# yangt1013/SPEINet

Hardware: AMD Instinct MI355X
Metric: deblurred 720p frames/sec (higher is better)
Workload: dtype f16 (correlation top2)

## Files before the change

speinet_amd/csrc/mlp_fused16.hip:

```cpp
#include "common.h"
#include <type_traits>

namespace {

constexpr int D = 256, HID = 512, MT = 128;
constexpr int RT = MT / 32;
constexpr int PA = 2 * D + 16;

template <typename LP>
struct MlpParams {
    const float* x;
    float* out;
    const LP* w1;
    const float* b1;
    const LP* w2;
    const float* b2;
    long long* stamps;
    int M;
};

typedef float f32x2 __attribute__((ext_vector_type(2)));

__device__ __forceinline__ f32x2 gelu2(f32x2 v) {
    const f32x2 u = v * v;
    f32x2 q = u * -1.419582270e-09f + 1.126438985e-07f;
    q = q * u + -3.898368825e-06f;
    q = q * u + 7.838465745e-05f;
    q = q * u + -1.034571474e-03f;
    q = q * u + 9.623637850e-03f;
    q = q * u + -6.612132016e-02f;
    q = q * u + 3.988274675e-01f;
    const f32x2 g = v * (v * q + 0.5f);
    f32x2 r;
    r[0] = fabsf(v[0]) < 4.0f ? g[0] : fmaxf(v[0], 0.f);
    r[1] = fabsf(v[1]) < 4.0f ? g[1] : fmaxf(v[1], 0.f);
    return r;
}

__device__ __forceinline__ f32x2 gelu2c(f32x2 v) {
    f32x2 c;
    c[0] = __builtin_amdgcn_fmed3f(v[0], -4.0f, 4.0f);
    c[1] = __builtin_amdgcn_fmed3f(v[1], -4.0f, 4.0f);
    const f32x2 u = c * c;
    f32x2 q = u * -1.419582270e-09f + 1.126438985e-07f;
    q = q * u + -3.898368825e-06f;
    q = q * u + 7.838465745e-05f;
    q = q * u + -1.034571474e-03f;
    q = q * u + 9.623637850e-03f;
    q = q * u + -6.612132016e-02f;
    q = q * u + 3.988274675e-01f;
    return v * (c * q + 0.5f);
}

struct GeluK { f32x2 c[8]; f32x2 half; };
__device__ __forceinline__ f32x2 sgpr_pair(float v) {
    f32x2 r = {v, v};
    asm volatile("" : "+s"(r));
    return r;
}
__device__ __forceinline__ GeluK gelu_consts() {
    GeluK k;
    k.c[0] = sgpr_pair(-1.419582270e-09f); k.c[1] = sgpr_pair(1.126438985e-07f); k.c[2] = sgpr_pair(-3.898368825e-06f);
    k.c[3] = sgpr_pair(7.838465745e-05f);  k.c[4] = sgpr_pair(-1.034571474e-03f); k.c[5] = sgpr_pair(9.623637850e-03f);
    k.c[6] = sgpr_pair(-6.612132016e-02f); k.c[7] = sgpr_pair(3.988274675e-01f);
    k.half = sgpr_pair(0.5f);
    return k;
}
__device__ __forceinline__ f32x4 gelu4c(f32x4 v, const GeluK& k) {
    const f32x2 va = {v[0], v[1]}, vb = {v[2], v[3]};
    f32x2 ca, cb;
    ca[0] = __builtin_amdgcn_fmed3f(v[0], -4.0f, 4.0f); ca[1] = __builtin_amdgcn_fmed3f(v[1], -4.0f, 4.0f);
    cb[0] = __builtin_amdgcn_fmed3f(v[2], -4.0f, 4.0f); cb[1] = __builtin_amdgcn_fmed3f(v[3], -4.0f, 4.0f);
    const f32x2 ua = ca * ca, ub = cb * cb;
    f32x2 qa = __builtin_elementwise_fma(ua, k.c[0], k.c[1]), qb = __builtin_elementwise_fma(ub, k.c[0], k.c[1]);
#pragma unroll
    for (int j = 2; j < 8; ++j) {
        qa = __builtin_elementwise_fma(qa, ua, k.c[j]);
        qb = __builtin_elementwise_fma(qb, ub, k.c[j]);
    }
    qa = __builtin_elementwise_fma(ca, qa, k.half);
    qb = __builtin_elementwise_fma(cb, qb, k.half);
    const f32x2 ga = va * qa, gb = vb * qb;
    return f32x4{ga[0], ga[1], gb[0], gb[1]};
}

template <int CTRL>
__device__ __forceinline__ float dpp_add(float v) { return v + dpp_quad<CTRL>(v); }
__device__ __forceinline__ float sum16(float v) { return dpp_add<0x140>(dpp_add<0x141>(dpp_add<0x4E>(dpp_add<0xB1>(v)))); }

template <typename LP>
__global__ __launch_bounds__(512) void mlp_fused_kernel(const MlpParams<LP> p) {
    typedef typename lpv<LP>::x8 lp8;
    typedef typename lpv<LP>::x4 lp4;
    constexpr int RG = 8;
    extern __shared__ __attribute__((aligned(16))) unsigned char smem[];
    unsigned char* sa = smem;
    unsigned char* sh = smem + MT * PA;
    float* bias1 = reinterpret_cast<float*>(smem + 2 * MT * PA);

    const int tid = threadIdx.x, lane = tid & 63, wave = tid >> 6;
    const int fr = lane & 31, fk = lane >> 5;
    const int m0 = blockIdx.x * MT;
    const int et = fr & 3, ecol = (fr >> 2) * 4;

    SPEI_STAMP(p.stamps, 0);
    bias1[tid] = p.b1[tid];
    const int rot = blockIdx.x & 15, rotb = rot * 32;

    {
        const int l16 = tid & 15, rsub = tid >> 4;
        f32x4 xr[MT / 32][4];
#pragma unroll
        for (int b = 0; b < MT / 32; ++b) {
            const int m = min(m0 + b * 32 + rsub, p.M - 1);
#pragma unroll
            for (int j = 0; j < 4; ++j) xr[b][j] = reinterpret_cast<const f32x4*>(p.x + (size_t)m * D)[l16 + 16 * j];
        }
#pragma unroll
        for (int b = 0; b < MT / 32; ++b) {
            const int r = b * 32 + rsub;
            float s = 0.f;
#pragma unroll
            for (int j = 0; j < 4; ++j) s += (xr[b][j][0] + xr[b][j][1]) + (xr[b][j][2] + xr[b][j][3]);
            const float mean = sum16(s) * (1.0f / 256.0f);
            float ss = 0.f;
#pragma unroll
            for (int j = 0; j < 4; ++j) {
                xr[b][j] -= mean;
                ss += (xr[b][j][0] * xr[b][j][0] + xr[b][j][1] * xr[b][j][1]) + (xr[b][j][2] * xr[b][j][2] + xr[b][j][3] * xr[b][j][3]);
            }
            const float rstd = 1.0f / sqrtf(sum16(ss) * (1.0f / 256.0f) + 1e-5f);
#pragma unroll
            for (int j = 0; j < 4; ++j) {
                lp4 hv;
#pragma unroll
                for (int e = 0; e < 4; ++e) hv[e] = to_lp<LP>(xr[b][j][e] * rstd);
                *reinterpret_cast<lp4*>(sa + r * PA + (((l16 + 16 * j) * 8 - rotb) & 511)) = hv;
            }
        }
    }

    lp8 ring[RG];
    const LP* wptr = p.w1 + (size_t)wave * 16 * 512 + lane * 8;
#pragma unroll
    for (int d = 0; d < RG; ++d) ring[d] = *reinterpret_cast<const lp8*>(wptr + ((rot + d) & 15) * 512);
    f32x4 res[RT][4];
#pragma unroll
    for (int i = 0; i < RT; ++i)
#pragma unroll
        for (int k = 0; k < 4; ++k) {
            const int m = min(m0 + i * 32 + 8 * k + 4 * fk + et, p.M - 1);
            res[i][k] = *reinterpret_cast<const f32x4*>(p.x + (size_t)m * D + wave * 32 + ecol);
        }
    __builtin_amdgcn_sched_barrier(0);
    lds_barrier();
    SPEI_STAMP(p.stamps, 1);

    f32x16 acc2[RT];
    const unsigned char* abase = sa + fr * PA + fk * 16;
    const unsigned char* hbase = sh + fr * PA + fk * 16;
#pragma unroll
    for (int half = 0; half < 2; ++half) {
        f32x16 acc1[RT];
#pragma unroll
        for (int g = 0; g < 4; ++g) {
            const f32x4 bv = *reinterpret_cast<const f32x4*>(bias1 + half * 256 + wave * 32 + 8 * g + 4 * fk);
#pragma unroll
            for (int i = 0; i < RT; ++i)
#pragma unroll
                for (int e = 0; e < 4; ++e) acc1[i][4 * g + e] = bv[e];
        }
        lp8 tn[RT];
#pragma unroll
        for (int i = 0; i < RT; ++i) tn[i] = *reinterpret_cast<const lp8*>(abase + i * 32 * PA);
        const LP* wnext = p.w2 + (size_t)wave * 32 * 512 + (size_t)half * 16 * 512 + lane * 8;
#pragma unroll
        for (int s = 0; s < 16; ++s) {
            lp8 tc[RT];
#pragma unroll
            for (int i = 0; i < RT; ++i) tc[i] = tn[i];
            if (s + 1 < 16) {
#pragma unroll
                for (int i = 0; i < RT; ++i) tn[i] = *reinterpret_cast<const lp8*>(abase + i * 32 * PA + (s + 1) * 32);
            }
            const lp8 w = ring[s % RG];
            ring[s % RG] = s + RG < 16 ? *reinterpret_cast<const lp8*>(wptr + ((rot + s + RG) & 15) * 512)
                                       : *reinterpret_cast<const lp8*>(wnext + ((rot + s + RG - 16) & 15) * 512);
            __builtin_amdgcn_sched_barrier(0);
#pragma unroll
            for (int i = 0; i < RT; ++i) acc1[i] = mfma16(w, tc[i], acc1[i]);
            __builtin_amdgcn_sched_barrier(0);
        }
        SPEI_STAMP(p.stamps, 2 + 3 * half);
        if (half == 0) {
            const float bias = p.b2[wave * 32 + fr];
#pragma unroll
            for (int i = 0; i < RT; ++i)
#pragma unroll
                for (int k = 0; k < 4; ++k) {
                    float a[4] = {res[i][k][0], res[i][k][1], res[i][k][2], res[i][k][3]};
                    quad_transpose4(a[0], a[1], a[2], a[3], et);
#pragma unroll
                    for (int e = 0; e < 4; ++e) acc2[i][4 * k + e] = a[e] + bias;
                }
        } else {
            lds_barrier();
        }
#pragma unroll
        for (int g = 0; g < 4; ++g) {
#pragma unroll
            for (int i = 0; i < RT; ++i) {
                const f32x2 g01 = gelu2c(f32x2{acc1[i][4 * g], acc1[i][4 * g + 1]});
                const f32x2 g23 = gelu2c(f32x2{acc1[i][4 * g + 2], acc1[i][4 * g + 3]});
                lp4 hv;
                hv[0] = to_lp<LP>(g01[0]); hv[1] = to_lp<LP>(g01[1]); hv[2] = to_lp<LP>(g23[0]); hv[3] = to_lp<LP>(g23[1]);
                *reinterpret_cast<lp4*>(sh + (i * 32 + fr) * PA + (((wave * 32 + 8 * g + 4 * fk) * 2 - rotb) & 511)) = hv;
            }
        }
        lds_barrier();
        SPEI_STAMP(p.stamps, 3 + 3 * half);
        wptr = wnext;
        const LP* wafter = p.w1 + (size_t)(8 + wave) * 16 * 512 + lane * 8;
#pragma unroll
        for (int i = 0; i < RT; ++i) tn[i] = *reinterpret_cast<const lp8*>(hbase + i * 32 * PA);
#pragma unroll
        for (int s = 0; s < 16; ++s) {
            lp8 tc[RT];
#pragma unroll
            for (int i = 0; i < RT; ++i) tc[i] = tn[i];
            if (s + 1 < 16) {
#pragma unroll
                for (int i = 0; i < RT; ++i) tn[i] = *reinterpret_cast<const lp8*>(hbase + i * 32 * PA + (s + 1) * 32);
            }
            const lp8 w = ring[s % RG];
            if (s + RG < 16) ring[s % RG] = *reinterpret_cast<const lp8*>(wptr + ((rot + s + RG) & 15) * 512);
            else if (half == 0) ring[s % RG] = *reinterpret_cast<const lp8*>(wafter + ((rot + s + RG - 16) & 15) * 512);
            __builtin_amdgcn_sched_barrier(0);
#pragma unroll
            for (int i = 0; i < RT; ++i) acc2[i] = mfma16(tc[i], w, acc2[i]);
            __builtin_amdgcn_sched_barrier(0);
        }
        SPEI_STAMP(p.stamps, 4 + 3 * half);
        wptr = wafter;
    }

#pragma unroll
    for (int i = 0; i < RT; ++i) {
#pragma unroll
        for (int k = 0; k < 4; ++k) {
            float a[4];
#pragma unroll
            for (int e = 0; e < 4; ++e) a[e] = acc2[i][4 * k + e];
            quad_transpose4(a[0], a[1], a[2], a[3], et);
            const int m = m0 + i * 32 + 8 * k + 4 * fk + et;
            if (m < p.M) *reinterpret_cast<f32x4*>(p.out + (size_t)m * D + wave * 32 + ecol) = f32x4{a[0], a[1], a[2], a[3]};
        }
    }
    SPEI_STAMP(p.stamps, 8);
}


constexpr int MP = 96;
constexpr int RP3 = MP / 32;
constexpr int SLABP = MP * PA;

template <typename LP>
__global__ __launch_bounds__(512) void mlp_pipe_kernel(const MlpParams<LP> p, const int ntiles, const int stagger) {
    typedef typename lpv<LP>::x8 lp8;
    typedef typename lpv<LP>::x4 lp4;
    constexpr int RG = 8;
    extern __shared__ __attribute__((aligned(16))) unsigned char smem[];
    unsigned char* const sb = smem + SLABP;
    float* bias1 = reinterpret_cast<float*>(smem + 3 * SLABP);

    const int tid = threadIdx.x, lane = tid & 63, wave = __builtin_amdgcn_readfirstlane(tid >> 6);
    const int fr = lane & 31, fk = lane >> 5;
    const int l16 = tid & 15, rsub = tid >> 4;

    SPEI_STAMP(p.stamps, 0); SPEI_STAMP_CLK(p.stamps, 8 + 0);
    spei_stagger_start(ntiles, stagger);
    bias1[tid] = p.b1[tid];
    const float bias2 = p.b2[wave * 32 + fr];
    const __amdgpu_buffer_rsrc_t rs1 = __builtin_amdgcn_make_buffer_rsrc(const_cast<LP*>(p.w1), 0, HID * D * 2, 0x00020000);
    const __amdgpu_buffer_rsrc_t rs2 = __builtin_amdgcn_make_buffer_rsrc(const_cast<LP*>(p.w2), 0, HID * D * 2, 0x00020000);
    const int lane16 = lane * 16;
    const int fbase[4] = {wave * 16, (8 + wave) * 16, wave * 32, wave * 32 + 16};
    auto wload = [&](int ph, int kstep) -> lp8 {
        return __builtin_bit_cast(lp8, __builtin_amdgcn_raw_buffer_load_b128(ph < 2 ? rs1 : rs2, lane16, (fbase[ph] + kstep) * 1024, 0));
    };

    const GeluK gk = gelu_consts();
    int tile = blockIdx.x;
    f32x4 xr[RP3][4];
    float lnm[RP3], lns[RP3];
    auto x_load = [&](int t, int b, int j) {
        const int m = min(t * MP + b * 32 + rsub, p.M - 1);
        xr[b][j] = reinterpret_cast<const f32x4*>(p.x + (size_t)m * D)[l16 + 16 * j];
    };
    auto ln_slice = [&](int b, int sub, unsigned char* dst, int rb) {
#pragma clang fp contract(off)
        if (sub == 0) {
            float s = 0.f;
#pragma unroll
            for (int j = 0; j < 4; ++j) s += (xr[b][j][0] + xr[b][j][1]) + (xr[b][j][2] + xr[b][j][3]);
            lnm[b] = sum16(s) * (1.0f / 256.0f);
        } else if (sub == 1) {
            float ss = 0.f;
#pragma unroll
            for (int j = 0; j < 4; ++j) {
                xr[b][j] -= lnm[b];
                ss += __builtin_fmaf(xr[b][j][1], xr[b][j][1], xr[b][j][0] * xr[b][j][0]) + __builtin_fmaf(xr[b][j][3], xr[b][j][3], xr[b][j][2] * xr[b][j][2]);
            }
            lns[b] = ss;
        } else if (sub == 2) {
            lns[b] = 1.0f / sqrtf(__builtin_fmaf(sum16(lns[b]), 1.0f / 256.0f, 1e-5f));
        } else {
            const int r = b * 32 + rsub;
#pragma unroll
            for (int j = 0; j < 4; ++j) {
                lp4 hv;
#pragma unroll
                for (int e = 0; e < 4; ++e) hv[e] = to_lp<LP>(xr[b][j][e] * lns[b]);
                *reinterpret_cast<lp4*>(dst + r * PA + (((l16 + 16 * j) * 8 - rb) & 511)) = hv;
            }
        }
    };

    int rot = tile & 15;
#pragma unroll
    for (int b = 0; b < RP3; ++b)
#pragma unroll
        for (int j = 0; j < 4; ++j) x_load(tile, b, j);
    lp8 ring[RG];
#pragma unroll
    for (int d = 0; d < RG; ++d) ring[d] = wload(0, (rot + d) & 15);
#pragma unroll
    for (int b = 0; b < RP3; ++b)
#pragma unroll
        for (int sub = 0; sub < 4; ++sub) ln_slice(b, sub, smem, rot * 32);
    __builtin_amdgcn_sched_barrier(0);
    lds_barrier();
    SPEI_STAMP(p.stamps, 1); SPEI_STAMP_CLK(p.stamps, 8 + 1);

    const unsigned range = (unsigned)p.M * (D * 4u);
    const __amdgpu_buffer_rsrc_t rsx = __builtin_amdgcn_make_buffer_rsrc(const_cast<float*>(p.x), 0, (int)range, 0x00020000);
    const __amdgpu_buffer_rsrc_t rso = __builtin_amdgcn_make_buffer_rsrc(p.out, 0, (int)range, 0x00020000);
    const unsigned voff_row = fk * 4096 + fr * 4;
    f32x16 acc2[RP3];
#pragma unroll
    for (int i = 0; i < RP3; ++i)
#pragma unroll
        for (int r = 0; r < 16; ++r) acc2[i][r] = 0.f;
    int cur = 0;
    bool first = true;
    for (; tile < ntiles; tile += gridDim.x) {
        unsigned char* const sa = smem + (cur ? 2 * SLABP : 0);
        unsigned char* const sc = smem + (cur ? 0 : 2 * SLABP);
        const int tnext = tile + gridDim.x;
        const int rotn = tnext & 15, rotb = rot * 32;
        auto wfrag = [&](int q) -> lp8 {
            return wload((q >> 4) & 3, ((q >= 64 ? rotn : rot) + (q & 15)) & 15);
        };
        auto gemm = [&](auto phc, const unsigned char* src, f32x16 (&acc)[RP3], auto weights_are_a, auto&& filler) {
            constexpr int ph = decltype(phc)::value;
            const unsigned char* base = src + fr * PA + fk * 16;
            lp8 tn[RP3];
#pragma unroll
            for (int i = 0; i < RP3; ++i) tn[i] = *reinterpret_cast<const lp8*>(base + i * 32 * PA);
#pragma unroll
            for (int s = 0; s < 16; ++s) {
                lp8 tc[RP3];
#pragma unroll
                for (int i = 0; i < RP3; ++i) tc[i] = tn[i];
                if (s + 1 < 16) {
#pragma unroll
                    for (int i = 0; i < RP3; ++i) tn[i] = *reinterpret_cast<const lp8*>(base + i * 32 * PA + (s + 1) * 32);
                }
                const lp8 w = ring[(ph * 16 + s) % RG];
                ring[(ph * 16 + s) % RG] = wfrag(ph * 16 + s + RG);
                __builtin_amdgcn_sched_barrier(0);
#pragma unroll
                for (int i = 0; i < RP3; ++i) {
                    if constexpr (decltype(weights_are_a)::value) acc[i] = mfma16(w, tc[i], acc[i]);
                    else acc[i] = mfma16(tc[i], w, acc[i]);
                }
                filler(s);
#pragma unroll
                for (int i = 0; i < RP3; ++i) asm volatile("" : "+v"(acc[i]));
                __builtin_amdgcn_sched_barrier(0);
            }
        };
        auto gelu_slice = [&](const f32x16 (&acc)[RP3], int s, unsigned char* dst) {
            if (s < 4 * RP3) {
                const int i = s >> 2, g = s & 3;
                const f32x4 gv = gelu4c(f32x4{acc[i][4 * g], acc[i][4 * g + 1], acc[i][4 * g + 2], acc[i][4 * g + 3]}, gk);
                *reinterpret_cast<lp4*>(dst + (i * 32 + fr) * PA + (((wave * 32 + 8 * g + 4 * fk) * 2 - rotb) & 511)) = to_lp4<LP>(gv);
            }
        };
        auto init_rows = [&](f32x16 (&acc)[RP3], const float* b) {
#pragma unroll
            for (int g = 0; g < 4; ++g) {
                const f32x4 bv = *reinterpret_cast<const f32x4*>(b + wave * 32 + 8 * g + 4 * fk);
#pragma unroll
                for (int i = 0; i < RP3; ++i)
#pragma unroll
                    for (int e = 0; e < 4; ++e) acc[i][4 * g + e] = bv[e];
            }
        };

        const unsigned vthis = voff_row + (unsigned)tile * (MP * 1024u), vprev = vthis - gridDim.x * (MP * 1024u);
        f32x16 acc1a[RP3], acc1b[RP3];
        f32x16 res[RP3];
        init_rows(acc1a, bias1);
        gemm(std::integral_constant<int, 0>{}, sa, acc1a, std::true_type{}, [&](int s) {
            if (s < 4 * RP3) {
                const int i = s >> 2, k = s & 3;
                const unsigned vst = vprev + (i * 32 + 8 * k) * 1024u, vld = vthis + (i * 32 + 8 * k) * 1024u;
#pragma unroll
                for (int e = 0; e < 4; ++e) {
                    __builtin_amdgcn_raw_buffer_store_b32(__float_as_uint(acc2[i][4 * k + e]), rso, (int)(vst + e * 1024u), wave * 128, 0);
                    res[i][4 * k + e] = __uint_as_float(__builtin_amdgcn_raw_buffer_load_b32(rsx, (int)(vld + e * 1024u), wave * 128, 0));
                }
            }
        });
        if (first) { SPEI_STAMP(p.stamps, 2); SPEI_STAMP_CLK(p.stamps, 8 + 2); }
        init_rows(acc1b, bias1 + 256);
        gemm(std::integral_constant<int, 1>{}, sa, acc1b, std::true_type{}, [&](int s) {
            gelu_slice(acc1a, s, sb);
            if (s >= 4 * RP3) {
#pragma unroll
                for (int i = 0; i < RP3; ++i)
#pragma unroll
                    for (int e = 0; e < 4; ++e) acc2[i][4 * (s - 4 * RP3) + e] = res[i][4 * (s - 4 * RP3) + e] + bias2;
            }
        });
        lds_barrier();
        if (first) { SPEI_STAMP(p.stamps, 3); SPEI_STAMP_CLK(p.stamps, 8 + 3); }
        gemm(std::integral_constant<int, 2>{}, sb, acc2, std::false_type{}, [&](int s) {
            gelu_slice(acc1b, s, sa);
            if (s >= 4 && (s & 3) < 2) {
                x_load(tnext, (s >> 2) - 1, 2 * (s & 1));
                x_load(tnext, (s >> 2) - 1, 2 * (s & 1) + 1);
            }
        });
        lds_barrier();
        if (first) { SPEI_STAMP(p.stamps, 4); SPEI_STAMP_CLK(p.stamps, 8 + 4); }
        gemm(std::integral_constant<int, 3>{}, sa, acc2, std::false_type{}, [&](int s) {
            if (s < 4 * RP3) ln_slice(s >> 2, s & 3, sc, rotn * 32);
        });
        if (first) { SPEI_STAMP(p.stamps, 5); SPEI_STAMP_CLK(p.stamps, 8 + 5); }
        lds_barrier();
        if (first) { SPEI_STAMP(p.stamps, 6); SPEI_STAMP_CLK(p.stamps, 8 + 6); }
        first = false;
        cur ^= 1;
        rot = rotn;
    }
#pragma unroll
    for (int i = 0; i < RP3; ++i)
#pragma unroll
        for (int r = 0; r < 16; ++r)
            __builtin_amdgcn_raw_buffer_store_b32(__float_as_uint(acc2[i][r]), rso,
                                                  (int)(voff_row + (unsigned)(tile - (int)gridDim.x) * (MP * 1024u) +
                                                        (i * 32 + 8 * (r >> 2) + (r & 3)) * 1024u), wave * 128, 0);
    SPEI_STAMP(p.stamps, 7); SPEI_STAMP_CLK(p.stamps, 8 + 7);
}

}

template <typename LP>
static int mlp_launch(const float* x, float* out, const void* w1, const float* b1, const void* w2, const float* b2, int64_t M, hipStream_t st) {
    MlpParams<LP> p;
    p.x = x; p.out = out; p.w1 = (const LP*)w1; p.b1 = b1; p.w2 = (const LP*)w2; p.b2 = b2; p.M = (int)M;
    p.stamps = spei_stamp_buffer();
    static const int pipe = spei_knob("SPEI_MLP_PIPE", 1);
    if (pipe && M <= (1ll << 21)) {
        const int ntiles = cdiv(M, MP);
        const size_t lds = (size_t)3 * SLABP + HID * sizeof(float);
        ensure_dyn_lds<&mlp_pipe_kernel<LP>>(lds);
        static const int stagger = spei_knob("SPEI_PIPE_STAGGER", 0);
        hipLaunchKernelGGL(mlp_pipe_kernel<LP>, dim3(ntiles < spei_num_cus() ? ntiles : spei_num_cus()), dim3(512), lds, st, p, ntiles, stagger);
        SPEI_CHECK_LAUNCH("spei_mlp_fused16");
        return 0;
    }
    const size_t lds = (size_t)2 * MT * PA + HID * sizeof(float);
    ensure_dyn_lds<&mlp_fused_kernel<LP>>(lds);
    hipLaunchKernelGGL(mlp_fused_kernel<LP>, dim3(cdiv(M, MT)), dim3(512), lds, st, p);
    SPEI_CHECK_LAUNCH("spei_mlp_fused16");
    return 0;
}

extern "C" int spei_mlp_fused16(int fmt, const float* x, float* out, const void* w1_frag, const float* b1, const void* w2_frag,
                                const float* b2, int64_t M, spei_stream_t stream) {
    SPEI_REQUIRE(x && out && w1_frag && b1 && w2_frag && b2 && M > 0, "spei_mlp_fused16: bad arguments");
    SPEI_REQUIRE(fmt == SPEI_BF16 || fmt == SPEI_F16, "spei_mlp_fused16: fmt=%d", fmt);
    SPEI_REQUIRE(M < (1ll << 31), "spei_mlp_fused16: too many tokens");
    SPEI_REQUIRE(((uintptr_t)x | (uintptr_t)out | (uintptr_t)w1_frag | (uintptr_t)w2_frag) % 16 == 0, "spei_mlp_fused16: 16-byte alignment required");
    hipStream_t st = (hipStream_t)stream;
    if (fmt == SPEI_F16) return mlp_launch<_Float16>(x, out, w1_frag, b1, w2_frag, b2, M, st);
    return mlp_launch<__bf16>(x, out, w1_frag, b1, w2_frag, b2, M, st);
}
```

Baseline: 42.09.

## Stash fp32 residual input in LDS instead of reloading it from global

```diff
diff --git a/speinet_amd/csrc/mlp_fused16.hip b/speinet_amd/csrc/mlp_fused16.hip
--- a/speinet_amd/csrc/mlp_fused16.hip
+++ b/speinet_amd/csrc/mlp_fused16.hip
@@ -263,6 +263,9 @@
 constexpr int MP = 96;
 constexpr int RP3 = MP / 32;
 constexpr int SLABP = MP * PA;
+constexpr int RESROWS = 56;
+constexpr int IMGB = RESROWS * D * 4;
+static_assert((MP - RESROWS) * D * 4 <= SLABP, "the image's second part must fit a slab");
 
 template <typename LP>
 __global__ __launch_bounds__(512) void mlp_pipe_kernel(const MlpParams<LP> p, const int ntiles, const int stagger) {
@@ -270,8 +273,8 @@
     typedef typename lpv<LP>::x4 lp4;
     constexpr int RG = 8;
     extern __shared__ __attribute__((aligned(16))) unsigned char smem[];
-    unsigned char* const sb = smem + SLABP;
-    float* bias1 = reinterpret_cast<float*>(smem + 3 * SLABP);
+    unsigned char* const sb = smem + 2 * SLABP;
+    float* bias1 = reinterpret_cast<float*>(sb + IMGB);
 
     const int tid = threadIdx.x, lane = tid & 63, wave = __builtin_amdgcn_readfirstlane(tid >> 6);
     const int fr = lane & 31, fk = lane >> 5;
@@ -304,12 +307,18 @@
 #pragma unroll
             for (int j = 0; j < 4; ++j) s += (xr[b][j][0] + xr[b][j][1]) + (xr[b][j][2] + xr[b][j][3]);
             lnm[b] = sum16(s) * (1.0f / 256.0f);
+            const int r = b * 32 + rsub;
+            if (r < RESROWS) {
+#pragma unroll
+                for (int j = 0; j < 4; ++j) *reinterpret_cast<f32x4*>(sb + r * (D * 4) + (l16 + 16 * j) * 16) = xr[b][j];
+            }
         } else if (sub == 1) {
             float ss = 0.f;
 #pragma unroll
             for (int j = 0; j < 4; ++j) {
-                xr[b][j] -= lnm[b];
-                ss += __builtin_fmaf(xr[b][j][1], xr[b][j][1], xr[b][j][0] * xr[b][j][0]) + __builtin_fmaf(xr[b][j][3], xr[b][j][3], xr[b][j][2] * xr[b][j][2]);
+                const f32x4 c = xr[b][j] - lnm[b];
+                if (b == 0) xr[b][j] = c;
+                ss += __builtin_fmaf(c[1], c[1], c[0] * c[0]) + __builtin_fmaf(c[3], c[3], c[2] * c[2]);
             }
             lns[b] = ss;
         } else if (sub == 2) {
@@ -318,9 +327,10 @@
             const int r = b * 32 + rsub;
 #pragma unroll
             for (int j = 0; j < 4; ++j) {
+                const f32x4 c = b == 0 ? xr[b][j] : xr[b][j] - lnm[b];
                 lp4 hv;
 #pragma unroll
-                for (int e = 0; e < 4; ++e) hv[e] = to_lp<LP>(xr[b][j][e] * lns[b]);
+                for (int e = 0; e < 4; ++e) hv[e] = to_lp<LP>(c[e] * lns[b]);
                 *reinterpret_cast<lp4*>(dst + r * PA + (((l16 + 16 * j) * 8 - rb) & 511)) = hv;
             }
         }
@@ -343,7 +353,6 @@
     SPEI_STAMP(p.stamps, 1); SPEI_STAMP_CLK(p.stamps, 8 + 1);
 
     const unsigned range = (unsigned)p.M * (D * 4u);
-    const __amdgpu_buffer_rsrc_t rsx = __builtin_amdgcn_make_buffer_rsrc(const_cast<float*>(p.x), 0, (int)range, 0x00020000);
     const __amdgpu_buffer_rsrc_t rso = __builtin_amdgcn_make_buffer_rsrc(p.out, 0, (int)range, 0x00020000);
     const unsigned voff_row = fk * 4096 + fr * 4;
     f32x16 acc2[RP3];
@@ -354,8 +363,8 @@
     int cur = 0;
     bool first = true;
     for (; tile < ntiles; tile += gridDim.x) {
-        unsigned char* const sa = smem + (cur ? 2 * SLABP : 0);
-        unsigned char* const sc = smem + (cur ? 0 : 2 * SLABP);
+        unsigned char* const sa = smem + (cur ? SLABP : 0);
+        unsigned char* const sc = smem + (cur ? 0 : SLABP);
         const int tnext = tile + gridDim.x;
         const int rotn = tnext & 15, rotb = rot * 32;
         auto wfrag = [&](int q) -> lp8 {
@@ -412,21 +421,36 @@
         f32x16 acc1a[RP3], acc1b[RP3];
         f32x16 res[RP3];
         init_rows(acc1a, bias1);
+#pragma unroll
+        for (int b = RESROWS / 32; b < RP3; ++b) {
+            const int r = b * 32 + rsub;
+            if (r >= RESROWS) {
+#pragma unroll
+                for (int j = 0; j < 4; ++j) *reinterpret_cast<f32x4*>(sc + (r - RESROWS) * (D * 4) + (l16 + 16 * j) * 16) = xr[b][j];
+            }
+        }
         gemm(std::integral_constant<int, 0>{}, sa, acc1a, std::true_type{}, [&](int s) {
             if (s < 4 * RP3) {
                 const int i = s >> 2, k = s & 3;
-                const unsigned vst = vprev + (i * 32 + 8 * k) * 1024u, vld = vthis + (i * 32 + 8 * k) * 1024u;
+                const unsigned vst = vprev + (i * 32 + 8 * k) * 1024u;
 #pragma unroll
                 for (int e = 0; e < 4; ++e) {
                     __builtin_amdgcn_raw_buffer_store_b32(__float_as_uint(acc2[i][4 * k + e]), rso, (int)(vst + e * 1024u), wave * 128, 0);
-                    res[i][4 * k + e] = __uint_as_float(__builtin_amdgcn_raw_buffer_load_b32(rsx, (int)(vld + e * 1024u), wave * 128, 0));
+                    if (i * 32 + 8 * k < RESROWS) res[i][4 * k + e] = *reinterpret_cast<const float*>(sb + voff_row + wave * 128 + (i * 32 + 8 * k + e) * 1024);
                 }
             }
         });
+        lds_barrier();
         if (first) { SPEI_STAMP(p.stamps, 2); SPEI_STAMP_CLK(p.stamps, 8 + 2); }
         init_rows(acc1b, bias1 + 256);
         gemm(std::integral_constant<int, 1>{}, sa, acc1b, std::true_type{}, [&](int s) {
             gelu_slice(acc1a, s, sb);
+            if (s < (MP - RESROWS) / 8) {
+                const int row = RESROWS + 8 * s, i = row >> 5, k = (row >> 3) & 3;
+#pragma unroll
+                for (int e = 0; e < 4; ++e)
+                    res[i][4 * k + e] = *reinterpret_cast<const float*>(sc + voff_row + wave * 128 + (8 * s + e) * 1024);
+            }
             if (s >= 4 * RP3) {
 #pragma unroll
                 for (int i = 0; i < RP3; ++i)
@@ -475,7 +499,8 @@
     static const int pipe = spei_knob("SPEI_MLP_PIPE", 1);
     if (pipe && M <= (1ll << 21)) {
         const int ntiles = cdiv(M, MP);
-        const size_t lds = (size_t)3 * SLABP + HID * sizeof(float);
+        static_assert(IMGB >= SLABP && 2 * SLABP + IMGB + HID * sizeof(float) <= 160 * 1024, "slabs + fp32 image + bias exceed a CU's LDS");
+        const size_t lds = (size_t)2 * SLABP + IMGB + HID * sizeof(float);
         ensure_dyn_lds<&mlp_pipe_kernel<LP>>(lds);
         static const int stagger = spei_knob("SPEI_PIPE_STAGGER", 0);
         hipLaunchKernelGGL(mlp_pipe_kernel<LP>, dim3(ntiles < spei_num_cus() ? ntiles : spei_num_cus()), dim3(512), lds, st, p, ntiles, stagger);
```

Result: no change. 42.38 (median of 6 runs) (+0.7%).
